# tjuDavidWang/MARL-UAVs-Targets-Tracking

Hardware: NVIDIA B200
Metric: agent-steps/s (higher is better)
Workload: dtype f64

## Files before the change

### marl_uavs_targets_tracking_b200/csrc/common.cuh

```cuda
#pragma once
#include <cuda_runtime.h>
#include <math.h>
#include <stdint.h>
#include <stdio.h>
#include <stdlib.h>
#include <string.h>

#include "../../include/uavsim.h"
#include "philox.cuh"

#define PMI_NT 256

enum { ST_REW, ST_TT, ST_BP, ST_DUP, ST_COV, ST_CMAX, ST_ENVS, ST_PMI_OOR, STAT_W };

static thread_local char g_err[512] = "";
#define SET_ERR(...) snprintf(g_err, sizeof(g_err), __VA_ARGS__)
#define CUDA_TRY(expr)                                                                     \
  do {                                                                                     \
    cudaError_t _e = (expr);                                                               \
    if (_e != cudaSuccess) {                                                               \
      SET_ERR("%s failed: %s (%s:%d)", #expr, cudaGetErrorString(_e), __FILE__, __LINE__); \
      return (int)_e;                                                                      \
    }                                                                                      \
  } while (0)

struct GuardK {
  float t2_up, t2_dn, c1, c0;
};

struct TileBand {
  float r, Cp, Hp, Cd, Hd, Cc, Hc, pad;
};

struct KParams {
  int n, m, na, num_steps;
  int64_t E;
  int64_t env_id_offset;
  double x_max, y_max;
  double dtv_u, dtv_t;
  double dt, uav_h_max;
  double dc, dp, two_dp;
  double tv, uv;
  double tv_over_uv;
  double s_dp_le, s_dp_lt, s_dc_le, s_2dp_le;
  double alpha, beta, gamma;
  double tt_hi;
  double dup_lo;
  double inv_dp, inv_dc, inv_na, inv_tt_hi, inv_dup_span;
  double cx, cy, rmax;
  float f_dp, f_dcmv;
  GuardK g_dp, g_2dp, g_dc, g_pf;
  float r_fast;
  float r_tile;
  TileBand tb[2];
  float dp_f, inv_dp_f, inv_dc_f, inv_na_f, tt_hi_f, inv_tt_hi_f, dup_lo_f, inv_dup_span_f, alpha_f, beta_f, gamma_f;
  float k_ex1_f, tv_over_uv_f, cx_f, cy_f;
  float dtv_u_f;
  const double *sincos_tab;
  int *fast_ctr;
};

struct PmiDev {
  int H;
  const float *w0, *b0, *w1t, *b1, *w2;
  float b2;
};

typedef void (*StepKernelFn)(const KParams, const UavSimBuffers, const double *, int64_t, int64_t, int, int, double,
                             int, long long *);
struct ActEntry;
typedef void (*FastKernelFn)(const KParams, const UavSimBuffers, const ActEntry *, int64_t, int64_t, int, double, int,
                             long long *);

typedef void (*SmallKernelFn)(const KParams, const UavSimBuffers, const ActEntry *, int64_t, int64_t, int, double, int,
                              long long *, int, uint64_t, uint32_t);

struct PmiTcDev;

struct uavsim {
  UavSimParams hp;
  KParams kp;
  UavSimBuffers buf;
  bool bound;
  int device, sm_count;
  int64_t E;
  double *d_dth;
  long long *d_stats;
  double *d_stats8;
  double *h_stats8;
  int stat_slots;
// ... 80 lines not shown
```

### marl_uavs_targets_tracking_b200/csrc/step_fast_kernel.cuh

```cuda
#pragma once
#include "common.cuh"
#include "fast_math.cuh"
#include <stddef.h>
#include "step_kernel.cuh"

#define FAST_NT 64

struct ActEntry {
  double dth;
  float cd, sd;
};

struct __align__(16) SlotRec {
  float4 pos;
  float4 hd;
  float2 a;
  float2 pad;
};
struct __align__(16) TSlot {
  float4 pos;
  float4 vel;
};

template <int N, int M, bool AUX>
struct __align__(128) FastSmem {
  double ux[N], uy[N], uh[N];
  double tx[M], ty[M], th[M];
  int32_t ua[N], act[N];
  double oux[N], ouy[N], ouh[N];
  double otx[M], oty[M], oth[M];
  int32_t oua[N];
  SlotRec slotn[N / 2];
  SlotRec sloto[N / 2];
  TSlot tslot[M / 2];
  double xo[N], yo[N];
  float raw[N];
  int32_t tcnt[AUX ? M : 1];
  uint32_t cover[2][2];
  uint32_t rmax[2];
  unsigned long long mbar;
  long long next_k;
};
static_assert(sizeof(SlotRec) == 48 && sizeof(TSlot) == 32, "slot layout");

__device__ __forceinline__ void sf_expect_tx(uint32_t bar, uint32_t bytes) {
  asm volatile("mbarrier.arrive.expect_tx.shared::cta.b64 _, [%0], %1;" ::"r"(bar), "r"(bytes) : "memory");
}
__device__ __forceinline__ void sf_bulk_g2s(uint32_t dst, const void *src, uint32_t bytes, uint32_t bar) {
  asm volatile("cp.async.bulk.shared::cluster.global.mbarrier::complete_tx::bytes [%0], [%1], %2, [%3];"
               ::"r"(dst), "l"(src), "r"(bytes), "r"(bar) : "memory");
}
__device__ __forceinline__ void sf_bulk_s2g(void *dst, uint32_t src, uint32_t bytes) {
  asm volatile("cp.async.bulk.global.shared::cta.bulk_group [%0], [%1], %2;" ::"l"(dst), "r"(src), "r"(bytes) : "memory");
}
__device__ __forceinline__ uint32_t sf_smem(const void *p) { return (uint32_t)__cvta_generic_to_shared(p); }
__device__ __forceinline__ void sf_mbar_wait(uint32_t bar, uint32_t parity) {
  uint32_t done = 0;
  for (uint32_t spin = 0; !done; spin++) {
    asm volatile(
        "{\n\t.reg .pred P1;\n\t"
        "mbarrier.try_wait.parity.shared::cta.b64 P1, [%1], %2, %3;\n\t"
        "selp.b32 %0, 1, 0, P1;\n\t}"
        : "=r"(done)
        : "r"(bar), "r"(parity), "r"(20000u)
        : "memory");
    if (spin > (1u << 22)) __trap();
  }
}

__device__ __forceinline__ uint64_t f2_sub(uint64_t a, uint64_t b) {
  uint64_t d;
  asm("sub.f32x2 %0, %1, %2;" : "=l"(d) : "l"(a), "l"(b));
  return d;
}
__device__ __forceinline__ uint64_t f2_fma(uint64_t a, uint64_t b, uint64_t c) {
  uint64_t d;
  asm("fma.rn.f32x2 %0, %1, %2, %3;" : "=l"(d) : "l"(a), "l"(b), "l"(c));
  return d;
}
__device__ __forceinline__ uint64_t f2_add(uint64_t a, uint64_t b) {
  uint64_t d;
  asm("add.f32x2 %0, %1, %2;" : "=l"(d) : "l"(a), "l"(b));
  return d;
}
__device__ __forceinline__ uint64_t f2_mul(uint64_t a, uint64_t b) {
  uint64_t d;
  asm("mul.f32x2 %0, %1, %2;" : "=l"(d) : "l"(a), "l"(b));
  return d;
}
__device__ __forceinline__ float f2_lo(uint64_t v) { return __uint_as_float((uint32_t)v); }
__device__ __forceinline__ float f2_hi(uint64_t v) { return __uint_as_float((uint32_t)(v >> 32)); }
__device__ __forceinline__ uint64_t sf_le2(float a0, float a1, float b) {
  uint32_t lo, hi;
  asm("{\n\t.reg .pred p, q;\n\t"
      "setp.le.f32 p, %2, %4;\n\t"
      "setp.le.f32 q, %3, %4;\n\t"
      "selp.b32 %0, 0x3f800000, 0, p;\n\t"
      "selp.b32 %1, 0x3f800000, 0, q;\n\t}"
      : "=r"(lo), "=r"(hi) : "f"(a0), "f"(a1), "f"(b));
  return (uint64_t)lo | ((uint64_t)hi << 32);
}
__device__ __forceinline__ float sf_le(float a, float b) { return (a <= b) ? 1.0f : 0.0f; }
__device__ __forceinline__ int sf_msb(uint32_t w) {
  int r;
  asm("bfind.u32 %0, %1;" : "=r"(r) : "r"(w));
  return r;
}
__device__ __forceinline__ float sf_rcp(float x) {
  float r;
  asm("rcp.approx.ftz.f32 %0, %1;" : "=f"(r) : "f"(x));
  return r;
}

template <bool TWO, int STRIDE>
__device__ __forceinline__ void prefilter64(const void *__restrict__ pf, float xf, float yf, float thrA, float thrB,
                                            uint32_t &aE, uint32_t &aO, uint32_t &bE, uint32_t &bO) {
  const uint64_t xf2 = pack2(xf, xf), yf2 = pack2(yf, yf), nA = pack2(-thrA, -thrA), nB = pack2(-thrB, -thrB);
  const unsigned char *base = reinterpret_cast<const unsigned char *>(pf);
  uint32_t ae = 0, ao = 0, be = 0, bo = 0;
#ifndef FAST_PF_UNROLL
#define FAST_PF_UNROLL 8
#endif
#pragma unroll 1
  for (int k = 0; k < 32; k += FAST_PF_UNROLL) {
#pragma unroll
    for (int u = 0; u < FAST_PF_UNROLL; u++) {
      const ulonglong2 p = *reinterpret_cast<const ulonglong2 *>(base + (k + u) * STRIDE);
      const uint64_t dx = f2_sub(p.x, xf2), dy = f2_sub(p.y, yf2);
      const uint64_t tA = f2_fma(dx, dx, f2_fma(dy, dy, nA));
      ae = __funnelshift_l((uint32_t)tA, ae, 1);
      ao = __funnelshift_l((uint32_t)(tA >> 32), ao, 1);
      if (TWO) {
        const uint64_t tB = f2_fma(dx, dx, f2_fma(dy, dy, nB));
        be = __funnelshift_l((uint32_t)tB, be, 1);
        bo = __funnelshift_l((uint32_t)(tB >> 32), bo, 1);
      }
    }
  }
  aE = __brev(ae); aO = __brev(ao);
// ... 187 lines not shown
      const float dx = r[0] - W.xf, dy = r[2] - W.yf;
      const float s = fmaf(dx, dx, dy * dy);
      if (s > T2_hi) continue;
      if (s > T2_lo && !(sf_exact_pair(S.oux[2 * b + par], S.ouy[2 * b + par], W.xi, W.yi, s_2dp_le, s_2dp_le) & 1)) continue;
      dp[par] |= bit;
      dup += fast_ex2f(fmaf(fast_sqrtf(s), k_ex1, k_ex0));
      if (s <= Tp_hi) {
        bool in = true;
        if (s > Tp_lo) in = sf_exact_pair(S.oux[2 * b + par], S.ouy[2 * b + par], W.xi, W.yi, s_dp_le, s_dp_le) & 1;
        if (in) nb[par] |= bit;
      }
    }
  }
  O->dup = dup; O->nbE = nb[0]; O->nbO = nb[1]; O->dpE = dp[0]; O->dpO = dp[1];
}


#ifndef FAST_LOAD_WARP
#define FAST_LOAD_WARP 1
#endif
#ifndef FAST_COV_THREAD
#define FAST_COV_THREAD 32
#endif
#ifndef FAST_CTAS_PER_SM
#define FAST_CTAS_PER_SM 14
#endif
template <int N, int M, bool AUX>
__global__ void __launch_bounds__(FAST_NT, FAST_CTAS_PER_SM)
uavsim_step_fast_kernel(const KParams P, const UavSimBuffers B, const ActEntry *__restrict__ act_tab, int64_t env_begin,
                        int64_t env_count, int mode, double coop, int done_flag, long long *__restrict__ stats) {
  static_assert(N == 64 && M == 64 && FAST_NT == 64, "one thread per UAV and per target");
  typedef FastSmem<N, M, AUX> SmemT;
  static_assert(offsetof(SmemT, sloto) - offsetof(SmemT, slotn) == sizeof(SlotRec) * (N / 2), "record offset");
  static_assert(sizeof(SlotRec) * N >= sizeof(float) * 12 * N && sizeof(TSlot) * (M / 2) >= sizeof(float) * 4 * N, "output staging");
  extern __shared__ __align__(128) unsigned char fast_smem_raw[];
  SmemT &S = *reinterpret_cast<SmemT *>(fast_smem_raw);
  float *const s_obs = reinterpret_cast<float *>(S.slotn);
  float *const s_rew = reinterpret_cast<float *>(S.tslot);
  const int t = threadIdx.x, lane = t & 31, warp = t >> 5;
  const uint32_t bar = sf_smem(&S.mbar);
  constexpr uint32_t IN_BYTES = 3 * N * 8 + 3 * M * 8 + 2 * N * 4;
  constexpr uint32_t OLD_OFF = (uint32_t)(sizeof(SlotRec) * (N / 2));
  const bool pmi_pending = (mode == UAVSIM_MODE_PMI) && (coop != 0.0);

  auto issue_loads = [&](int64_t e) {
    sf_expect_tx(bar, IN_BYTES);
    sf_bulk_g2s(sf_smem(S.ux), B.ux + e * N, N * 8, bar);
    sf_bulk_g2s(sf_smem(S.uy), B.uy + e * N, N * 8, bar);
    sf_bulk_g2s(sf_smem(S.uh), B.uh + e * N, N * 8, bar);
    sf_bulk_g2s(sf_smem(S.tx), B.tx + e * M, M * 8, bar);
    sf_bulk_g2s(sf_smem(S.ty), B.ty + e * M, M * 8, bar);
    sf_bulk_g2s(sf_smem(S.th), B.th + e * M, M * 8, bar);
    sf_bulk_g2s(sf_smem(S.ua), B.ua + e * N, N * 4, bar);
    sf_bulk_g2s(sf_smem(S.act), B.actions + e * N, N * 4, bar);
  };

  if (t == 0) {
    mbar_init(bar, 1);
    asm volatile("fence.mbarrier_init.release.cluster;" ::: "memory");
  }
  __syncthreads();
  if (warp == 0 && (int64_t)blockIdx.x < env_count) {
    if (elect_one()) issue_loads(env_begin + blockIdx.x);
  }

  const int64_t plane = P.E * N;
  const float inv_dp_f = P.inv_dp_f, inv_dc_f = P.inv_dc_f, inv_na_f = P.inv_na_f;
  const float k_ex0 = 1.4426950408889634f, k_ex1 = P.k_ex1_f;
  int fx_r = 0, fx_tt = 0, fx_bp = 0, fx_dup = 0;
  long long fxs_r = 0, fxs_tt = 0, fxs_bp = 0, fxs_dup = 0;
  long long st_cov = 0, st_envs = 0;
  int st_cmax = 0;
  uint32_t trips = 0;
  uint32_t parity = 0;
  const int ih = t >> 1, ic = t & 1;
  const int ihx = ih + ic;

  for (int64_t k = blockIdx.x, k_next = 0; k < env_count; k = k_next) {
    const int64_t e = env_begin + k;
    sf_mbar_wait(bar, parity);
    parity ^= 1;

    double t_x = S.tx[t], t_y = S.ty[t], t_h = S.th[t];
    float t_vx, t_vy;
    {
      double sh, ch;
      heading_sincos(t_h, P.sincos_tab, sh, ch);
      t_x += P.dtv_t * ch;
      t_y += P.dtv_t * sh;
      if (0 > t_y || t_y > P.y_max) { t_h = -t_h; sh = -sh; }
      else if (t_x < 0 || t_x > P.x_max) { t_h = (t_h > 0) ? (PI_D - t_h) : (-PI_D - t_h); ch = -ch; }
      t_vx = (float)ch * P.tv_over_uv_f; t_vy = (float)sh * P.tv_over_uv_f;
    }
    const float txf = (float)(t_x - P.cx), tyf = (float)(t_y - P.cy);
    float rabs = fmaxf(fabsf(txf), fabsf(tyf));
    double xi, yi, hi;
    float xf, yf, chf, shf, xl, yl;
    const double xo_d = S.ux[t], yo_d = S.uy[t];
    const int a_old = S.ua[t], ai = S.act[t];
    float xof, yof, cof, sof;
    {
      double h = S.uh[t];
      double sh, ch;
      heading_sincos(h, P.sincos_tab, sh, ch);
      cof = (float)ch; sof = (float)sh;
      xof = (float)(xo_d - P.cx); yof = (float)(yo_d - P.cy);
      xi = xo_d + P.dtv_u * ch;
      yi = yo_d + P.dtv_u * sh;
      double dh;
      float cd, sd;
      if ((unsigned)ai < (unsigned)P.na) {
        const ActEntry en = act_tab[ai];
        dh = en.dth; cd = en.cd; sd = en.sd;
      } else {
        dh = P.dt * ((double)(2 * (ai + 1) - P.na - 1) * P.uav_h_max / (double)(P.na - 1));
        double sd_, cd_;
        sincos_shared(dh, &sd_, &cd_);
        cd = (float)cd_; sd = (float)sd_;
      }
      hi = wrap_heading(h + dh);
      chf = fmaf(cof, cd, -(sof * sd));
      shf = fmaf(sof, cd, cof * sd);
      xf = (float)(xi - P.cx); yf = (float)(yi - P.cy);
      xl = (float)((xi - P.cx) - (double)xf); yl = (float)((yi - P.cy) - (double)yf);
      rabs = fmaxf(fmaxf(rabs, fmaxf(fabsf(xf), fabsf(yf))), fmaxf(fabsf(xof), fabsf(yof)));
      if ((unsigned)ai >= 4096u || (unsigned)a_old >= 4096u) rabs = __int_as_float(0x7f800000);
      if (!(rabs == rabs)) rabs = __int_as_float(0x7f800000);
    }
    if (warp == 0) {
      if (elect_one()) asm volatile("cp.async.bulk.wait_group.read 0;" ::: "memory");
    }
    __syncthreads();
    {
      S.otx[t] = t_x; S.oty[t] = t_y; S.oth[t] = t_h;
      float *ts = reinterpret_cast<float *>(&S.tslot[ih]) + ic;
      ts[0] = txf; ts[2] = tyf; ts[4] = t_vx; ts[6] = t_vy;
      if (AUX) S.tcnt[t] = 0;
      S.xo[t] = xo_d; S.yo[t] = yo_d;
      float *so = reinterpret_cast<float *>(&S.sloto[ih]) + ic;
      so[0] = xof; so[2] = yof; so[4] = cof; so[6] = sof; so[8] = (float)a_old;
      S.oux[t] = xi; S.ouy[t] = yi; S.ouh[t] = hi; S.oua[t] = ai;
      float *sn = reinterpret_cast<float *>(&S.slotn[ih]) + ic;
      sn[0] = xf; sn[2] = yf; sn[4] = chf; sn[6] = shf; sn[8] = (float)ai;
    }
    {
      const uint32_t rm = __reduce_max_sync(0xffffffffu, __float_as_uint(rabs));
      if (lane == 0) S.rmax[warp] = rm;
    }
    __syncthreads();
    if (warp == FAST_LOAD_WARP) {
      if (elect_one()) {
        const int64_t kn = (int64_t)gridDim.x + (int64_t)atomicAdd(P.fast_ctr, 1);
        S.next_k = kn;
        if (kn < env_count) issue_loads(env_begin + kn);
      }
    }

    const float R = __uint_as_float(max(S.rmax[0], S.rmax[1]));
    const bool far_env = !(R <= P.r_fast);
    const bool near_origin = fabs(xi) < 2.0 && fabs(yi) < 2.0;
    const int64_t mrow_t = (e * N + t) * M, mrow_u = (e * N + t) * N;
    float o0, o1, o2, o3, o4, o5, o6, o7, o8, tt_f, dup_f;
    uint32_t nbE = 0, nbO = 0, cvE = 0, cvO = 0;
    uint32_t ncE = 0, ncO = 0;
    uint32_t cmE = 0, cmO = 0, dpE = 0, dpO = 0;
#ifdef FAST_ABL_NOPAIRS
    const bool exact = false;
    o0 = o1 = o2 = o3 = o4 = o5 = o6 = o7 = o8 = -1.f; tt_f = 0.f; dup_f = 0.f;
    if (far_env && near_origin) {
#else
    const bool exact = far_env || near_origin;
    if (!exact) {
#endif
      const float g_dp = fmaf(R, P.g_dp.c1, P.g_dp.c0), g_2dp = fmaf(R, P.g_2dp.c1, P.g_2dp.c0);
      const float ndtv_f = -P.dtv_u_f;
      const float g_dc = 2.0f * fmaf(R, P.g_dc.c1, P.g_dc.c0) + P.g_dc.c1 * fabsf(P.dtv_u_f);
      const float g_pf = fmaf(R, P.g_pf.c1, P.g_pf.c0);
      const float Tp_hi = __fadd_ru(P.g_dp.t2_up, g_dp), Tp_lo = __fadd_rd(P.g_dp.t2_dn, -g_dp);
      const float T2_hi = __fadd_ru(P.g_2dp.t2_up, g_2dp), T2_lo = __fadd_rd(P.g_2dp.t2_dn, -g_2dp);
      const float Tc_hi = __fadd_ru(P.g_dc.t2_up, g_dc), Tc_lo = __fadd_rd(P.g_dc.t2_dn, -g_dc);
      const float Tf_hi = __fadd_ru(P.g_pf.t2_up, g_pf);
      const uint64_t xf2 = pack2(xf, xf), yf2 = pack2(yf, yf);
      const WalkOwn WO = {xi, yi, xf, yf, t};

      uint32_t ccE, ccO;
      {
        uint32_t d0, d1;
        prefilter64<false, (int)sizeof(TSlot)>(S.tslot, xf, yf, Tp_hi, 0.f, cvE, cvO, d0, d1);
        float ox = 0, oy = 0, ovx = 0, ovy = 0, ttacc = 0, smax_t = 0;
#pragma unroll
        for (int par = 0; par < 2; par++) {
          uint32_t w = par ? cvO : cvE;
          const float *rec = reinterpret_cast<const float *>(S.tslot) + par;
#pragma unroll 1
          while (w) {
            const int b = sf_msb(w);
            w ^= 1u << b;
            const float *r = rec + 8 * b;
            const float dx = r[0] - xf, dy = r[2] - yf;
            const float s = fmaf(dx, dx, dy * dy);
            smax_t = fmaxf(smax_t, s);
            ox += dx; oy += dy; ovx += r[4]; ovy += r[6];
            ttacc = fmaf(fast_sqrtf(s), -inv_dp_f, ttacc);
          }
        }
        if (smax_t > Tp_lo) {
          TgtOut X;
          sf_targets_checked<N, M, AUX>(&S, WO, Tp_lo, P.s_dp_le, P.s_dp_lt, inv_dp_f, cvE, cvO, &X);
          ox = X.ox; oy = X.oy; ovx = X.ovx; ovy = X.ovy; ttacc = X.ttacc;
          cvE = X.cvE; cvO = X.cvO; ncE = X.ncE; ncO = X.ncO;
        }
        const int nobs = __popc(cvE) + __popc(cvO);
        if (nobs) {
          const float kf = (float)nobs, rk = sf_rcp(kf);
          o5 = fmaf(ox, rk, -xl) * inv_dp_f;
          o6 = fmaf(oy, rk, -yl) * inv_dp_f;
          o7 = fmaf(ovx, rk, -chf);
          o8 = fmaf(ovy, rk, -shf);
          tt_f = fmaf(2.0f, kf, ttacc);
        } else {
          o5 = o6 = o7 = o8 = -1.f;
          tt_f = 0.f;
        }
      }

      uint32_t d0_, d1_;
      prefilter64<false, (int)sizeof(SlotRec)>(S.slotn, xf, yf, Tf_hi, 0.f, ccE, ccO, d0_, d1_);
      const unsigned char *slot_new = reinterpret_cast<const unsigned char *>(S.slotn);
      const unsigned char *slot_old = reinterpret_cast<const unsigned char *>(S.sloto);
      {
        uint64_t sx = 0, sy = 0, sc = 0, ss = 0, sa = 0, cn = 0, dp2 = 0;
        float smax_c = 0.f, smax_d = 0.f, dmin_n = 3.0e38f;
        const float Tp_nx = __uint_as_float(__float_as_uint(Tp_hi) + 1u);
        const uint64_t tpn2 = pack2(Tp_nx, Tp_nx);
        const float nb_band = fmaxf(__fadd_ru(Tp_nx, -Tp_lo), 4.0f * (Tp_nx - Tp_hi));
        const uint64_t kx1 = pack2(k_ex1, k_ex1), kx0 = pack2(k_ex0, k_ex0);
        uint32_t w = ccE | ccO;
#pragma unroll 1
        while (w) {
          const int b = sf_msb(w);
          const uint32_t bit = 1u << b;
// ... 21 lines not shown
          sa = f2_fma(wh, aa, sa);
          cn = f2_add(cn, wh);
          if (AUX) { if (h0) cmE |= bit; if (h1) cmO |= bit; }
          const uint64_t n2 = f2_fma(ex, ex, f2_mul(ey, ey));
          const float n0 = f2_lo(n2), n1 = f2_hi(n2);
          const bool g0 = n0 <= T2_hi, g1 = n1 <= T2_hi;
          const uint64_t wg = pack2(g0 ? 1.0f : 0.0f, g1 ? 1.0f : 0.0f);
          {
            const uint64_t nw = f2_mul(n2, wg);
            smax_d = fmaxf(fmaxf(smax_d, f2_lo(nw)), f2_hi(nw));
          }
          const uint64_t arg = f2_fma(pack2(fast_sqrtf(n0), fast_sqrtf(n1)), kx1, kx0);
          dp2 = f2_fma(wg, pack2(fast_ex2f(f2_lo(arg)), fast_ex2f(f2_hi(arg))), dp2);
          if (AUX) { if (g0) dpE |= bit; if (g1) dpO |= bit; }
          {
            const uint64_t dn = f2_sub(n2, tpn2);
            const uint32_t m0 = (uint32_t)((int32_t)(uint32_t)dn >> 31), m1 = (uint32_t)((int32_t)(uint32_t)(dn >> 32) >> 31);
            nbE |= m0 & bit; nbO |= m1 & bit;
            dmin_n = fminf(fminf(dmin_n, fabsf(f2_lo(dn))), fabsf(f2_hi(dn)));
          }
        }
        float own_w, own_dx, own_dy, own_c, own_s, own_a;
        {
          const float *r = reinterpret_cast<const float *>(slot_new + (ic ? 0u : OLD_OFF) + 48 * ih) + ic;
          own_c = r[4]; own_s = r[6]; own_a = r[8];
          own_dx = own_c * (ic ? 0.0f : ndtv_f); own_dy = own_s * (ic ? 0.0f : ndtv_f);
          const float s_own = fmaf(own_dx, own_dx, own_dy * own_dy);
          own_w = sf_le(s_own, Tc_hi);
        }
        float tsx = f2_lo(sx) + f2_hi(sx), tsy = f2_lo(sy) + f2_hi(sy), tsc = f2_lo(sc) + f2_hi(sc);
        float tss = f2_lo(ss) + f2_hi(ss), tsa = f2_lo(sa) + f2_hi(sa), tcn = f2_lo(cn) + f2_hi(cn);
        if (smax_c > Tc_lo) {
          CommOut X;
          sf_comm_checked<N, M, AUX>(&S, WO, Tc_lo, Tc_hi, P.s_dc_le, ihx, ccE | ccO, &X);
          tsx = X.sx; tsy = X.sy; tsc = X.sc; tss = X.ss; tsa = X.sa; tcn = X.cn;
          if (AUX) { cmE = X.cmE; cmO = X.cmO; }
        }
        const float cntf = tcn - own_w;
        if (AUX) { if (ic) cmO &= ~(1u << ih); else cmE &= ~(1u << ih); }
        if (cntf > 0.5f) {
          const float rk = sf_rcp(cntf);
          o0 = fmaf(tsx - own_w * own_dx, rk, -xl) * inv_dc_f;
          o1 = fmaf(tsy - own_w * own_dy, rk, -yl) * inv_dc_f;
          o2 = fmaf(tsc - own_w * own_c, rk, -chf);
          o3 = fmaf(tss - own_w * own_s, rk, -shf);
          o4 = ((tsa - own_w * own_a) - cntf * (float)ai) * (rk * inv_na_f);
        } else {
          o0 = o1 = o2 = o3 = o4 = -1.f;
        }
        const uint32_t ownE = ic ? 0u : (1u << ih), ownO = ic ? (1u << ih) : 0u;
        float dup = (f2_lo(dp2) + f2_hi(dp2)) - fast_ex2f(fmaf(fast_sqrtf(0.f), k_ex1, k_ex0));
        nbE &= ~ownE; nbO &= ~ownO;
        if (AUX) { dpE &= ~ownE; dpO &= ~ownO; }
        if ((smax_d > T2_lo) || (dmin_n <= nb_band)) {
          DupOut X;
          sf_dup_checked<N, M, AUX>(&S, WO, T2_lo, T2_hi, Tp_lo, Tp_hi, P.s_2dp_le, P.s_dp_le, k_ex0, k_ex1, (ccE | ccO) & ~ownE,
                                    (ccE | ccO) & ~ownO, &X);
          dup = X.dup; nbE = X.nbE; nbO = X.nbO;
          if (AUX) { dpE = X.dpE; dpO = X.dpO; }
        }
        dup_f = -0.5f * dup;
      }
    }
    if (exact) {
      const ExactK XK = {P.s_dp_le, P.s_dp_lt, P.s_2dp_le, P.s_dc_le, P.dp, P.dc, P.two_dp, P.na};
      const MaskPtrs MP = {B.obs_mask, B.comm_mask, B.nbr_mask, B.dup_mask, B.cover_mask};
      FastAgent X;
      fast_agent_exact<N, M, AUX>(XK, MP, S, t, mrow_t, mrow_u, &X);
      o0 = X.ob[0]; o1 = X.ob[1]; o2 = X.ob[2]; o3 = X.ob[3]; o4 = X.ob[4];
      o5 = X.ob[5]; o6 = X.ob[6]; o7 = X.ob[7]; o8 = X.ob[8];
      tt_f = X.tt; dup_f = X.dup;
      nbE = X.nb[0]; nbO = X.nb[1]; cvE = X.cov[0]; cvO = X.cov[1];
    } else if (AUX && B.obs_mask) {
      for (int j = 0; j < 64; j++) {
        const int b = j >> 1;
        const uint8_t v = (((j & 1) ? cvO : cvE) >> b) & 1u;
        B.obs_mask[mrow_t + j] = v; B.cover_mask[mrow_t + j] = v & ~((((j & 1) ? ncO : ncE) >> b) & 1u);
        B.comm_mask[mrow_u + j] = (((j & 1) ? cmO : cmE) >> b) & 1u;
        B.nbr_mask[mrow_u + j] = (((j & 1) ? nbO : nbE) >> b) & 1u;
        B.dup_mask[mrow_u + j] = (((j & 1) ? dpO : dpE) >> b) & 1u;
      }
    }
    cvE &= ~ncE; cvO &= ~ncO;
    if (AUX && B.tracker_cnt) {
#pragma unroll
      for (int par = 0; par < 2; par++) {
        uint32_t w = par ? cvO : cvE;
        while (w) { const int b = sf_msb(w); w ^= 1u << b; atomicAdd(&S.tcnt[2 * b + par], 1); }
      }
    }
    {
      const uint32_t c0 = __reduce_or_sync(0xffffffffu, cvE), c1 = __reduce_or_sync(0xffffffffu, cvO);
      if (lane == 0) { S.cover[warp][0] = c0; S.cover[warp][1] = c1; }
    }

    float raw, ttn, bpn, dupn;
    {
      const float dbdr = fminf(P.cx_f - fabsf(xf), P.cy_f - fabsf(yf));
      bool inside = dbdr > 0.f;
      if (fabsf(dbdr) < 1e-3f) inside = 0 <= xi && xi <= P.x_max && 0 <= yi && yi <= P.y_max;
      const float bp = inside ? ((dbdr < P.dp_f) ? (-0.5f * (P.dp_f - dbdr) * inv_dp_f) : 0.0f) : -0.5f;
      ttn = fminf(fmaxf(tt_f, 0.0f), P.tt_hi_f) * P.inv_tt_hi_f;
      dupn = (fminf(fmaxf(dup_f, P.dup_lo_f), 0.0f) - P.dup_lo_f) * P.inv_dup_span_f - 1.0f;
      bpn = (fminf(fmaxf(bp, -0.5f), 0.0f) + 0.5f) * 2.0f - 1.0f;
      raw = fmaf(P.alpha_f, ttn, fmaf(P.beta_f, bpn, P.gamma_f * dupn));
      S.raw[t] = raw;
    }
    __syncthreads();
    k_next = S.next_k;

    {
      float *ob = s_obs + t * 12;
      reinterpret_cast<float4 *>(ob)[0] = make_float4(o0, o1, o2, o3);
      reinterpret_cast<float4 *>(ob)[1] = make_float4(o4, o5, o6, o7);
      reinterpret_cast<float4 *>(ob)[2] = make_float4(o8, (float)(xi * P.inv_dc), (float)(yi * P.inv_dc), (float)ai * inv_na_f);
      float r;
      const int64_t gi = e * N + t;
      if (mode == UAVSIM_MODE_SELF || coop == 0.0) {
        r = raw;
      } else if (mode == UAVSIM_MODE_MEAN) {
        float s = 0;
        const int cnt = __popc(nbE) + __popc(nbO);
        {
          uint32_t u = nbE | nbO;
          float s1 = 0;
          while (u) {
            const int b = sf_msb(u);
            const uint32_t bit = 1u << b;
            u ^= bit;
            const float2 rr = *reinterpret_cast<const float2 *>(&S.raw[2 * b]);
            s += (nbE & bit) ? rr.x : 0.0f;
            s1 += (nbO & bit) ? rr.y : 0.0f;
          }
          s += s1;
        }
        const float cf = (float)coop;
        r = cnt ? fmaf(1.0f - cf, raw, cf * s * sf_rcp((float)cnt)) : 0.0f;
      } else {
        r = 0.0f;
        B.raw[gi] = (double)raw;
        B.nbr_bits[gi * 2] = sf_interleave(nbE, nbO);
        B.nbr_bits[gi * 2 + 1] = 0;
      }
      r = fminf(fmaxf(r, -1.0f), 1.0f);
      s_rew[t] = r;
      s_rew[N + t] = ttn;
      s_rew[2 * N + t] = bpn;
      s_rew[3 * N + t] = dupn;
      if (!pmi_pending) fx_r += sf_fx(r);
      fx_tt += sf_fx(ttn); fx_bp += sf_fx(bpn); fx_dup += sf_fx(dupn);
      if ((++trips & 255u) == 0u) {
        fxs_r += fx_r; fxs_tt += fx_tt; fxs_bp += fx_bp; fxs_dup += fx_dup;
        fx_r = fx_tt = fx_bp = fx_dup = 0;
      }
      if (AUX && B.tracker_cnt) B.tracker_cnt[e * M + t] = S.tcnt[t];
    }
    asm volatile("fence.proxy.async.shared::cta;" ::: "memory");
    __syncthreads();
    if (warp == 0) {
      if (elect_one()) {
        sf_bulk_s2g(B.ux + e * N, sf_smem(S.oux), N * 8);
        sf_bulk_s2g(B.uy + e * N, sf_smem(S.ouy), N * 8);
        sf_bulk_s2g(B.uh + e * N, sf_smem(S.ouh), N * 8);
        sf_bulk_s2g(B.ua + e * N, sf_smem(S.oua), N * 4);
        sf_bulk_s2g(B.tx + e * M, sf_smem(S.otx), M * 8);
        sf_bulk_s2g(B.ty + e * M, sf_smem(S.oty), M * 8);
        sf_bulk_s2g(B.th + e * M, sf_smem(S.oth), M * 8);
        sf_bulk_s2g(B.obs + e * N * 12, sf_smem(s_obs), N * 48);
        if (!pmi_pending) sf_bulk_s2g(B.rew4 + e * N, sf_smem(s_rew), N * 4);
        sf_bulk_s2g(B.rew4 + plane + e * N, sf_smem(s_rew + N), N * 4);
        sf_bulk_s2g(B.rew4 + 2 * plane + e * N, sf_smem(s_rew + 2 * N), N * 4);
        sf_bulk_s2g(B.rew4 + 3 * plane + e * N, sf_smem(s_rew + 3 * N), N * 4);
        asm volatile("cp.async.bulk.commit_group;" ::: "memory");
      }
    }
    if (t == FAST_COV_THREAD) {
      const int c = __popc(S.cover[0][0] | S.cover[1][0]) + __popc(S.cover[0][1] | S.cover[1][1]);
      B.covered[e] = c;
      if (B.done) B.done[e] = done_flag;
      st_cov += c;
      st_cmax = max(st_cmax, c);
      st_envs++;
    }
  }
  __syncwarp();
  if (warp == 0) {
    if (elect_one()) asm volatile("cp.async.bulk.wait_group 0;" ::: "memory");
  }
  work_counter_leave(P.fast_ctr);
  stats_commit(stats + (size_t)blockIdx.x * STAT_W, fxs_r + fx_r, fxs_tt + fx_tt, fxs_bp + fx_bp, fxs_dup + fx_dup, st_cov,
               st_cmax, st_envs);
}
```

### marl_uavs_targets_tracking_b200/csrc/uavsim.cu

```cuda
#include <cfloat>
#include <cmath>
#include <mutex>
#include <vector>

#include "common.cuh"
#include "step_kernel.cuh"
#include "pmi_kernel.cuh"
#include "pmi_tc_kernel.cuh"
#include "step_fast_kernel.cuh"
#include "step_tile_kernel.cuh"
#include "step_small_kernel.cuh"
#include "aux_kernels.cuh"
#include "replay.cuh"

static double exact_sq_threshold(double thr, bool strict) {
  double s = thr * thr;
  auto ok = [&](double v) { double r = sqrt(v); return strict ? (r < thr) : (r <= thr); };
  while (!ok(s)) s = nextafter(s, -INFINITY);
  while (ok(nextafter(s, INFINITY))) s = nextafter(s, INFINITY);
  return s;
}

static int raise_dynamic_smem(const void *fn, int device, size_t bytes) {
  static struct { const void *fn; int device; size_t bytes; } seen[256];
// ... 117 lines not shown
  k.g_dc = make_guard(p->dc, k.rmax);
  {
    const double rmin = p->dp < p->dc ? p->dp : p->dc;
    double rf = 2e-6 * 16777216.0 * rmin;
    if (rf > k.rmax) rf = k.rmax;
    k.r_fast = (float)rf;
    k.r_tile = (float)(rf < 4096.0 ? rf : 4096.0);
    const double cmax = k.cx > k.cy ? k.cx : k.cy;
    const double rr[2] = {1.3 * cmax < k.r_tile ? 1.3 * cmax : (double)k.r_tile, (double)k.r_tile};
    for (int lv = 0; lv < 2; lv++) {
      auto band = [&](const GuardK &G, float &C, float &H) {
        const double gd = ((double)G.c1 * rr[lv] + (double)G.c0) * (1.0 + 1e-6);
        const double hi = (double)G.t2_up + gd, lo = (double)G.t2_dn - gd;
        C = (float)(0.5 * (hi + lo));
        const double hw = 0.5 * (hi - lo) + 2.4e-7 * fabs(hi) + fabs((double)C - 0.5 * (hi + lo));
        H = nextafterf((float)hw, INFINITY);
        if ((double)H < hw) H = nextafterf(H, INFINITY);
      };
      k.tb[lv].r = (float)rr[lv];
      if ((double)k.tb[lv].r > rr[lv]) k.tb[lv].r = nextafterf(k.tb[lv].r, 0.f);
      band(k.g_dp, k.tb[lv].Cp, k.tb[lv].Hp);
      band(k.g_2dp, k.tb[lv].Cd, k.tb[lv].Hd);
      band(k.g_dc, k.tb[lv].Cc, k.tb[lv].Hc);
      k.tb[lv].pad = 0.f;
    }
  }
  k.dp_f = (float)p->dp; k.inv_dp_f = (float)k.inv_dp; k.inv_dc_f = (float)k.inv_dc; k.inv_na_f = (float)k.inv_na;
  k.tt_hi_f = (float)k.tt_hi; k.inv_tt_hi_f = (float)k.inv_tt_hi; k.dup_lo_f = (float)k.dup_lo; k.inv_dup_span_f = (float)k.inv_dup_span;
  k.alpha_f = (float)k.alpha; k.beta_f = (float)k.beta; k.gamma_f = (float)k.gamma;
  k.k_ex1_f = (float)(-1.4426950408889634 / k.two_dp); k.tv_over_uv_f = (float)k.tv_over_uv;
  k.cx_f = (float)k.cx; k.cy_f = (float)k.cy;
  k.dtv_u_f = (float)k.dtv_u;
  {
    double tab[FM_TAB_SIZE * 2];
    fm_fill_table(tab);
    CUDA_TRY(cudaMalloc(&h->d_sctab, sizeof(tab)));
    CUDA_TRY(cudaMemcpy(h->d_sctab, tab, sizeof(tab), cudaMemcpyHostToDevice));
    k.sincos_tab = h->d_sctab;
    CUDA_TRY(cudaMalloc(&h->d_fast_ctr, 2 * sizeof(int)));
    CUDA_TRY(cudaMemset(h->d_fast_ctr, 0, 2 * sizeof(int)));
    k.fast_ctr = h->d_fast_ctr;
  }

  std::vector<double> dth_v(3 * (size_t)p->na);
  double *dth = dth_v.data();
  for (int a = 0; a < p->na; a++) {
    const int na1 = a + 1;
    const double rate = (double)(2 * na1 - p->na - 1) * p->uav_h_max / (double)(p->na - 1);
    dth[3 * a] = p->dt * rate;
    dth[3 * a + 1] = cos(dth[3 * a]);
    dth[3 * a + 2] = sin(dth[3 * a]);
  }
  CUDA_TRY(cudaMalloc(&h->d_dth, sizeof(double) * 3 * p->na));
  CUDA_TRY(cudaMemcpy(h->d_dth, dth, sizeof(double) * 3 * p->na, cudaMemcpyHostToDevice));
  {
    std::vector<ActEntry> tab(p->na);
    for (int a = 0; a < p->na; a++) { tab[a].dth = dth[3 * a]; tab[a].cd = (float)dth[3 * a + 1]; tab[a].sd = (float)dth[3 * a + 2]; }
    CUDA_TRY(cudaMalloc(&h->d_act, sizeof(ActEntry) * p->na));
    CUDA_TRY(cudaMemcpy(h->d_act, tab.data(), sizeof(ActEntry) * p->na, cudaMemcpyHostToDevice));
  }

  if (k.n == 64 && k.m == 64) { h->nt = UAVSIM_NT64; h->step_fn[0] = uavsim_step_kernel<64, 64, false, UAVSIM_NT64>; h->step_fn[1] = uavsim_step_kernel<64, 64, true, UAVSIM_NT64>; }
  else if (k.n == 10 && k.m == 10) { h->nt = 128; h->step_fn[0] = uavsim_step_kernel<10, 10, false, 128>; h->step_fn[1] = uavsim_step_kernel<10, 10, true, 128>; }
  else { h->nt = 128; h->step_fn[0] = uavsim_step_kernel<0, 0, false, 128>; h->step_fn[1] = uavsim_step_kernel<0, 0, true, 128>; }
  int epb = h->nt / p->n_uav;
  if (epb < 1) epb = 1;
  const bool fixed_shape = (k.n == 64 && k.m == 64) || (k.n == 10 && k.m == 10);
  if (!fixed_shape) {
    if ((int64_t)epb > n_envs) epb = (int)n_envs;
    while (epb > 1 && step_smem_bytes(k.n, k.m, k.na, epb) > 64 * 1024) epb--;
  }
  h->epb = epb;
  h->smem_step = step_smem_bytes(k.n, k.m, k.na, epb);
  if (h->smem_step > 227 * 1024) {
    SET_ERR("uavsim_create: n_uav=%d m_targets=%d needs %zu B shared memory per CTA", k.n, k.m, h->smem_step);
    return UAVSIM_ERR_UNSUPPORTED;
  }
  for (int v = 0; v < 2; v++) {
    int rc = raise_dynamic_smem((const void *)h->step_fn[v], device, h->smem_step);
    if (rc) return rc;
  }
  int occ = 1;
  CUDA_TRY(cudaOccupancyMaxActiveBlocksPerMultiprocessor(&occ, h->step_fn[0], h->nt, h->smem_step));
  if (occ < 1) occ = 1;
  h->grid_max = h->sm_count * occ;
  h->has_fast = (k.n == 64 && k.m == 64);
  if (h->has_fast) {
    h->fast_fn[0] = uavsim_step_fast_kernel<64, 64, false>;
    h->fast_fn[1] = uavsim_step_fast_kernel<64, 64, true>;
    h->smem_fast[0] = sizeof(FastSmem<64, 64, false>);
    h->smem_fast[1] = sizeof(FastSmem<64, 64, true>);
    for (int v = 0; v < 2; v++) {
      int rc = raise_dynamic_smem((const void *)h->fast_fn[v], device, h->smem_fast[v]);
      if (rc) return rc;
      int o = 1;
      CUDA_TRY(cudaOccupancyMaxActiveBlocksPerMultiprocessor(&o, h->fast_fn[v], FAST_NT, h->smem_fast[v]));
      h->fast_grid_max[v] = h->sm_count * (o < 1 ? 1 : o);
      if (h->fast_grid_max[v] > h->grid_max) h->grid_max = h->fast_grid_max[v];
    }
    h->tile_fn[0] = uavsim_step_tile_kernel<false>;
    h->tile_fn[1] = uavsim_step_tile_kernel<true>;
    h->smem_tile[0] = sizeof(TileSmem<false>);
    h->smem_tile[1] = sizeof(TileSmem<true>);
    for (int v = 0; v < 2; v++) {
      int rc = raise_dynamic_smem((const void *)h->tile_fn[v], device, h->smem_tile[v]);
      if (rc) return rc;
      int o = 1;
      CUDA_TRY(cudaOccupancyMaxActiveBlocksPerMultiprocessor(&o, h->tile_fn[v], TILE_NT, h->smem_tile[v]));
      h->tile_grid_max[v] = h->sm_count * (o < 1 ? 1 : o);
      if (h->tile_grid_max[v] > h->grid_max) h->grid_max = h->tile_grid_max[v];
    }
  }
  h->has_small = (k.n <= SMALL_MAX && k.m <= SMALL_MAX);
  int small_warps = 0;
  if (h->has_small) {
    h->small_fn[0] = uavsim_step_small_kernel<false>;
    h->small_fn[1] = uavsim_step_small_kernel<true>;
    for (int v = 0; v < 2; v++) {
      int o = 1;
      CUDA_TRY(cudaOccupancyMaxActiveBlocksPerMultiprocessor(&o, h->small_fn[v], SMALL_NT, 0));
      h->small_grid_max[v] = h->sm_count * (o < 1 ? 1 : o);
      if (h->small_grid_max[v] > small_warps) small_warps = h->small_grid_max[v];
    }
  }
// ... 634 lines not shown
```

Measured before the change: 10.09 billion.

## Add strip-grid target culling, smem action table, and reduce register pressure in fast kernel

Replaces the full 64-target prefilter scan with a per-env 1D strip grid on x and y. Each target sets bits in overlapping strip windows, and each UAV only tests targets whose bits survive in both its x and y strips. The action table moves into shared memory, per-thread stat accumulators become per-warp shared counters updated by warp reductions, and several live values (env index, own position, lane-local data) are reloaded from shared memory instead of held in registers. The likely aim is to cut per-UAV distance work and register pressure. The cost is shared atomics, extra syncs on strip zeroing, and more dynamic shared memory, which may lower occupancy.

```diff
diff --git a/marl_uavs_targets_tracking_b200/csrc/common.cuh b/marl_uavs_targets_tracking_b200/csrc/common.cuh
--- a/marl_uavs_targets_tracking_b200/csrc/common.cuh
+++ b/marl_uavs_targets_tracking_b200/csrc/common.cuh
@@ -56,6 +56,8 @@
   float dp_f, inv_dp_f, inv_dc_f, inv_na_f, tt_hi_f, inv_tt_hi_f, dup_lo_f, inv_dup_span_f, alpha_f, beta_f, gamma_f;
   float k_ex1_f, tv_over_uv_f, cx_f, cy_f;
   float dtv_u_f;
+  float tg_q, tg_inv_x, tg_off_x, tg_inv_y, tg_off_y;
+  int tg_nx, tg_ny;
   const double *sincos_tab;
   int *fast_ctr;
 };
diff --git a/marl_uavs_targets_tracking_b200/csrc/step_fast_kernel.cuh b/marl_uavs_targets_tracking_b200/csrc/step_fast_kernel.cuh
--- a/marl_uavs_targets_tracking_b200/csrc/step_fast_kernel.cuh
+++ b/marl_uavs_targets_tracking_b200/csrc/step_fast_kernel.cuh
@@ -5,6 +5,7 @@
 #include "step_kernel.cuh"
 
 #define FAST_NT 64
+#define FAST_STRIPS 32
 
 struct ActEntry {
   double dth;
@@ -33,6 +34,7 @@
   SlotRec slotn[N / 2];
   SlotRec sloto[N / 2];
   TSlot tslot[M / 2];
+  uint2 xwin[FAST_STRIPS], ywin[FAST_STRIPS];
   double xo[N], yo[N];
   float raw[N];
   int32_t tcnt[AUX ? M : 1];
@@ -40,6 +42,10 @@
   uint32_t rmax[2];
   unsigned long long mbar;
   long long next_k;
+  long long cur_e;
+  long long fx[2][4];
+  long long cov_sum;
+  int cov_max, n_env;
 };
 static_assert(sizeof(SlotRec) == 48 && sizeof(TSlot) == 32, "slot layout");
 
@@ -105,6 +111,9 @@
   int r;
   asm("bfind.u32 %0, %1;" : "=r"(r) : "r"(w));
   return r;
+}
+__device__ __forceinline__ int sf_strip(float u, float inv, float off, int nc) {
+  return min(max(__float2int_rd(fmaf(u, inv, off)), 0), nc - 1);
 }
 __device__ __forceinline__ float sf_rcp(float x) {
   float r;
@@ -358,6 +367,8 @@
   static_assert(N == 64 && M == 64 && FAST_NT == 64, "one thread per UAV and per target");
   typedef FastSmem<N, M, AUX> SmemT;
   static_assert(offsetof(SmemT, sloto) - offsetof(SmemT, slotn) == sizeof(SlotRec) * (N / 2), "record offset");
+  static_assert(offsetof(SmemT, xwin) % 16 == 0 && offsetof(SmemT, ywin) == offsetof(SmemT, xwin) + 8 * FAST_STRIPS &&
+                2 * FAST_STRIPS * 8 <= 16 * FAST_NT, "strip windows are zeroed with one 16-byte store per thread");
   static_assert(sizeof(SlotRec) * N >= sizeof(float) * 12 * N && sizeof(TSlot) * (M / 2) >= sizeof(float) * 4 * N, "output staging");
   extern __shared__ __align__(128) unsigned char fast_smem_raw[];
   SmemT &S = *reinterpret_cast<SmemT *>(fast_smem_raw);
@@ -381,6 +392,11 @@
     sf_bulk_g2s(sf_smem(S.act), B.actions + e * N, N * 4, bar);
   };
 
+  ActEntry *const s_act = reinterpret_cast<ActEntry *>(fast_smem_raw + sizeof(SmemT));
+  for (int a = t; a < P.na; a += FAST_NT) s_act[a] = act_tab[a];
+  if (t < FAST_STRIPS) reinterpret_cast<uint4 *>(S.xwin)[t] = make_uint4(0, 0, 0, 0);
+  if (lane == 0) for (int k = 0; k < 4; k++) S.fx[warp][k] = 0;
+  if (t == FAST_COV_THREAD) { S.cov_sum = 0; S.cov_max = 0; S.n_env = 0; }
   if (t == 0) {
     mbar_init(bar, 1);
     asm volatile("fence.mbarrier_init.release.cluster;" ::: "memory");
@@ -393,17 +409,11 @@
   const int64_t plane = P.E * N;
   const float inv_dp_f = P.inv_dp_f, inv_dc_f = P.inv_dc_f, inv_na_f = P.inv_na_f;
   const float k_ex0 = 1.4426950408889634f, k_ex1 = P.k_ex1_f;
-  int fx_r = 0, fx_tt = 0, fx_bp = 0, fx_dup = 0;
-  long long fxs_r = 0, fxs_tt = 0, fxs_bp = 0, fxs_dup = 0;
-  long long st_cov = 0, st_envs = 0;
-  int st_cmax = 0;
-  uint32_t trips = 0;
   uint32_t parity = 0;
   const int ih = t >> 1, ic = t & 1;
   const int ihx = ih + ic;
 
   for (int64_t k = blockIdx.x, k_next = 0; k < env_count; k = k_next) {
-    const int64_t e = env_begin + k;
     sf_mbar_wait(bar, parity);
     parity ^= 1;
 
@@ -421,6 +431,7 @@
     const float txf = (float)(t_x - P.cx), tyf = (float)(t_y - P.cy);
     float rabs = fmaxf(fabsf(txf), fabsf(tyf));
     double xi, yi, hi;
+    bool near_origin;
     float xf, yf, chf, shf, xl, yl;
     const double xo_d = S.ux[t], yo_d = S.uy[t];
     const int a_old = S.ua[t], ai = S.act[t];
@@ -436,7 +447,7 @@
       double dh;
       float cd, sd;
       if ((unsigned)ai < (unsigned)P.na) {
-        const ActEntry en = act_tab[ai];
+        const ActEntry en = s_act[ai];
         dh = en.dth; cd = en.cd; sd = en.sd;
       } else {
         dh = P.dt * ((double)(2 * (ai + 1) - P.na - 1) * P.uav_h_max / (double)(P.na - 1));
@@ -449,6 +460,7 @@
       shf = fmaf(sof, cd, cof * sd);
       xf = (float)(xi - P.cx); yf = (float)(yi - P.cy);
       xl = (float)((xi - P.cx) - (double)xf); yl = (float)((yi - P.cy) - (double)yf);
+      near_origin = fabs(xi) < 2.0 && fabs(yi) < 2.0;
       rabs = fmaxf(fmaxf(rabs, fmaxf(fabsf(xf), fabsf(yf))), fmaxf(fabsf(xof), fabsf(yof)));
       if ((unsigned)ai >= 4096u || (unsigned)a_old >= 4096u) rabs = __int_as_float(0x7f800000);
       if (!(rabs == rabs)) rabs = __int_as_float(0x7f800000);
@@ -458,9 +470,22 @@
     }
     __syncthreads();
     {
+      if (t == 0) S.cur_e = env_begin + k;
       S.otx[t] = t_x; S.oty[t] = t_y; S.oth[t] = t_h;
       float *ts = reinterpret_cast<float *>(&S.tslot[ih]) + ic;
       ts[0] = txf; ts[2] = tyf; ts[4] = t_vx; ts[6] = t_vy;
+      {
+        const float q = P.tg_q;
+        const uint32_t bit = 1u << ih;
+        const int gx1 = sf_strip(txf + q, P.tg_inv_x, P.tg_off_x, P.tg_nx);
+#pragma unroll 1
+        for (int g = sf_strip(txf - q, P.tg_inv_x, P.tg_off_x, P.tg_nx); g <= gx1; g++)
+          atomicOr(reinterpret_cast<uint32_t *>(&S.xwin[g]) + ic, bit);
+        const int gy1 = sf_strip(tyf + q, P.tg_inv_y, P.tg_off_y, P.tg_ny);
+#pragma unroll 1
+        for (int g = sf_strip(tyf - q, P.tg_inv_y, P.tg_off_y, P.tg_ny); g <= gy1; g++)
+          atomicOr(reinterpret_cast<uint32_t *>(&S.ywin[g]) + ic, bit);
+      }
       if (AUX) S.tcnt[t] = 0;
       S.xo[t] = xo_d; S.yo[t] = yo_d;
       float *so = reinterpret_cast<float *>(&S.sloto[ih]) + ic;
@@ -484,8 +509,7 @@
 
     const float R = __uint_as_float(max(S.rmax[0], S.rmax[1]));
     const bool far_env = !(R <= P.r_fast);
-    const bool near_origin = fabs(xi) < 2.0 && fabs(yi) < 2.0;
-    const int64_t mrow_t = (e * N + t) * M, mrow_u = (e * N + t) * N;
+    const float *const own_new = reinterpret_cast<const float *>(&S.slotn[ih]) + ic;
     float o0, o1, o2, o3, o4, o5, o6, o7, o8, tt_f, dup_f;
     uint32_t nbE = 0, nbO = 0, cvE = 0, cvO = 0;
     uint32_t ncE = 0, ncO = 0;
@@ -507,12 +531,27 @@
       const float Tc_hi = __fadd_ru(P.g_dc.t2_up, g_dc), Tc_lo = __fadd_rd(P.g_dc.t2_dn, -g_dc);
       const float Tf_hi = __fadd_ru(P.g_pf.t2_up, g_pf);
       const uint64_t xf2 = pack2(xf, xf), yf2 = pack2(yf, yf);
-      const WalkOwn WO = {xi, yi, xf, yf, t};
+      auto own_walk = [&]() { return WalkOwn{S.oux[t], S.ouy[t], xf, yf, t}; };
 
       uint32_t ccE, ccO;
       {
-        uint32_t d0, d1;
-        prefilter64<false, (int)sizeof(TSlot)>(S.tslot, xf, yf, Tp_hi, 0.f, cvE, cvO, d0, d1);
+        {
+          const uint2 wx = S.xwin[sf_strip(xf, P.tg_inv_x, P.tg_off_x, P.tg_nx)];
+          const uint2 wy = S.ywin[sf_strip(yf, P.tg_inv_y, P.tg_off_y, P.tg_ny)];
+          const uint64_t nT = pack2(-Tp_hi, -Tp_hi);
+          uint32_t w = (wx.x & wy.x) | (wx.y & wy.y);
+#pragma unroll 1
+          while (w) {
+            const int b = sf_msb(w);
+            const uint32_t bit = 1u << b;
+            w ^= bit;
+            const ulonglong2 p = *reinterpret_cast<const ulonglong2 *>(&S.tslot[b].pos);
+            const uint64_t dx = f2_sub(p.x, xf2), dy = f2_sub(p.y, yf2);
+            const uint64_t tA = f2_fma(dx, dx, f2_fma(dy, dy, nT));
+            cvE |= (uint32_t)((int32_t)(uint32_t)tA >> 31) & bit;
+            cvO |= (uint32_t)((int32_t)(uint32_t)(tA >> 32) >> 31) & bit;
+          }
+        }
         float ox = 0, oy = 0, ovx = 0, ovy = 0, ttacc = 0, smax_t = 0;
 #pragma unroll
         for (int par = 0; par < 2; par++) {
@@ -532,7 +571,7 @@
         }
         if (smax_t > Tp_lo) {
           TgtOut X;
-          sf_targets_checked<N, M, AUX>(&S, WO, Tp_lo, P.s_dp_le, P.s_dp_lt, inv_dp_f, cvE, cvO, &X);
+          sf_targets_checked<N, M, AUX>(&S, own_walk(), Tp_lo, P.s_dp_le, P.s_dp_lt, inv_dp_f, cvE, cvO, &X);
           ox = X.ox; oy = X.oy; ovx = X.ovx; ovy = X.ovy; ttacc = X.ttacc;
           cvE = X.cvE; cvO = X.cvO; ncE = X.ncE; ncO = X.ncO;
         }
@@ -620,7 +659,7 @@
         float tss = f2_lo(ss) + f2_hi(ss), tsa = f2_lo(sa) + f2_hi(sa), tcn = f2_lo(cn) + f2_hi(cn);
         if (smax_c > Tc_lo) {
           CommOut X;
-          sf_comm_checked<N, M, AUX>(&S, WO, Tc_lo, Tc_hi, P.s_dc_le, ihx, ccE | ccO, &X);
+          sf_comm_checked<N, M, AUX>(&S, own_walk(), Tc_lo, Tc_hi, P.s_dc_le, ihx, ccE | ccO, &X);
           tsx = X.sx; tsy = X.sy; tsc = X.sc; tss = X.ss; tsa = X.sa; tcn = X.cn;
           if (AUX) { cmE = X.cmE; cmO = X.cmO; }
         }
@@ -628,11 +667,12 @@
         if (AUX) { if (ic) cmO &= ~(1u << ih); else cmE &= ~(1u << ih); }
         if (cntf > 0.5f) {
           const float rk = sf_rcp(cntf);
-          o0 = fmaf(tsx - own_w * own_dx, rk, -xl) * inv_dc_f;
-          o1 = fmaf(tsy - own_w * own_dy, rk, -yl) * inv_dc_f;
-          o2 = fmaf(tsc - own_w * own_c, rk, -chf);
-          o3 = fmaf(tss - own_w * own_s, rk, -shf);
-          o4 = ((tsa - own_w * own_a) - cntf * (float)ai) * (rk * inv_na_f);
+          const float xl2 = (float)((S.oux[t] - P.cx) - (double)xf), yl2 = (float)((S.ouy[t] - P.cy) - (double)yf);
+          o0 = fmaf(tsx - own_w * own_dx, rk, -xl2) * inv_dc_f;
+          o1 = fmaf(tsy - own_w * own_dy, rk, -yl2) * inv_dc_f;
+          o2 = fmaf(tsc - own_w * own_c, rk, -own_new[4]);
+          o3 = fmaf(tss - own_w * own_s, rk, -own_new[6]);
+          o4 = ((tsa - own_w * own_a) - cntf * own_new[8]) * (rk * inv_na_f);
         } else {
           o0 = o1 = o2 = o3 = o4 = -1.f;
         }
@@ -642,7 +682,7 @@
         if (AUX) { dpE &= ~ownE; dpO &= ~ownO; }
         if ((smax_d > T2_lo) || (dmin_n <= nb_band)) {
           DupOut X;
-          sf_dup_checked<N, M, AUX>(&S, WO, T2_lo, T2_hi, Tp_lo, Tp_hi, P.s_2dp_le, P.s_dp_le, k_ex0, k_ex1, (ccE | ccO) & ~ownE,
+          sf_dup_checked<N, M, AUX>(&S, own_walk(), T2_lo, T2_hi, Tp_lo, Tp_hi, P.s_2dp_le, P.s_dp_le, k_ex0, k_ex1, (ccE | ccO) & ~ownE,
                                     (ccE | ccO) & ~ownO, &X);
           dup = X.dup; nbE = X.nbE; nbO = X.nbO;
           if (AUX) { dpE = X.dpE; dpO = X.dpO; }
@@ -650,6 +690,8 @@
         dup_f = -0.5f * dup;
       }
     }
+    const int64_t e = S.cur_e;
+    const int64_t mrow_t = (e * N + t) * M, mrow_u = (e * N + t) * N;
     if (exact) {
       const ExactK XK = {P.s_dp_le, P.s_dp_lt, P.s_2dp_le, P.s_dc_le, P.dp, P.dc, P.two_dp, P.na};
       const MaskPtrs MP = {B.obs_mask, B.comm_mask, B.nbr_mask, B.dup_mask, B.cover_mask};
@@ -683,6 +725,7 @@
     }
 
     float raw, ttn, bpn, dupn;
+    xi = S.oux[t]; yi = S.ouy[t];
     {
       const float dbdr = fminf(P.cx_f - fabsf(xf), P.cy_f - fabsf(yf));
       bool inside = dbdr > 0.f;
@@ -696,12 +739,13 @@
     }
     __syncthreads();
     k_next = S.next_k;
+    if (t < FAST_STRIPS) reinterpret_cast<uint4 *>(S.xwin)[t] = make_uint4(0, 0, 0, 0);
 
     {
       float *ob = s_obs + t * 12;
       reinterpret_cast<float4 *>(ob)[0] = make_float4(o0, o1, o2, o3);
       reinterpret_cast<float4 *>(ob)[1] = make_float4(o4, o5, o6, o7);
-      reinterpret_cast<float4 *>(ob)[2] = make_float4(o8, (float)(xi * P.inv_dc), (float)(yi * P.inv_dc), (float)ai * inv_na_f);
+      reinterpret_cast<float4 *>(ob)[2] = make_float4(o8, (float)(xi * P.inv_dc), (float)(yi * P.inv_dc), (float)S.oua[t] * inv_na_f);
       float r;
       const int64_t gi = e * N + t;
       if (mode == UAVSIM_MODE_SELF || coop == 0.0) {
@@ -735,11 +779,11 @@
       s_rew[N + t] = ttn;
       s_rew[2 * N + t] = bpn;
       s_rew[3 * N + t] = dupn;
-      if (!pmi_pending) fx_r += sf_fx(r);
-      fx_tt += sf_fx(ttn); fx_bp += sf_fx(bpn); fx_dup += sf_fx(dupn);
-      if ((++trips & 255u) == 0u) {
-        fxs_r += fx_r; fxs_tt += fx_tt; fxs_bp += fx_bp; fxs_dup += fx_dup;
-        fx_r = fx_tt = fx_bp = fx_dup = 0;
+      {
+        const int w_r = __reduce_add_sync(0xffffffffu, pmi_pending ? 0 : sf_fx(r));
+        const int w_tt = __reduce_add_sync(0xffffffffu, sf_fx(ttn)), w_bp = __reduce_add_sync(0xffffffffu, sf_fx(bpn));
+        const int w_dup = __reduce_add_sync(0xffffffffu, sf_fx(dupn));
+        if (lane == 0) { S.fx[warp][0] += w_r; S.fx[warp][1] += w_tt; S.fx[warp][2] += w_bp; S.fx[warp][3] += w_dup; }
       }
       if (AUX && B.tracker_cnt) B.tracker_cnt[e * M + t] = S.tcnt[t];
     }
@@ -747,28 +791,31 @@
     __syncthreads();
     if (warp == 0) {
       if (elect_one()) {
-        sf_bulk_s2g(B.ux + e * N, sf_smem(S.oux), N * 8);
-        sf_bulk_s2g(B.uy + e * N, sf_smem(S.ouy), N * 8);
-        sf_bulk_s2g(B.uh + e * N, sf_smem(S.ouh), N * 8);
-        sf_bulk_s2g(B.ua + e * N, sf_smem(S.oua), N * 4);
-        sf_bulk_s2g(B.tx + e * M, sf_smem(S.otx), M * 8);
-        sf_bulk_s2g(B.ty + e * M, sf_smem(S.oty), M * 8);
-        sf_bulk_s2g(B.th + e * M, sf_smem(S.oth), M * 8);
-        sf_bulk_s2g(B.obs + e * N * 12, sf_smem(s_obs), N * 48);
-        if (!pmi_pending) sf_bulk_s2g(B.rew4 + e * N, sf_smem(s_rew), N * 4);
-        sf_bulk_s2g(B.rew4 + plane + e * N, sf_smem(s_rew + N), N * 4);
-        sf_bulk_s2g(B.rew4 + 2 * plane + e * N, sf_smem(s_rew + 2 * N), N * 4);
-        sf_bulk_s2g(B.rew4 + 3 * plane + e * N, sf_smem(s_rew + 3 * N), N * 4);
+        const int64_t o = S.cur_e * N;
+        sf_bulk_s2g(B.ux + o, sf_smem(S.oux), N * 8);
+        sf_bulk_s2g(B.uy + o, sf_smem(S.ouy), N * 8);
+        sf_bulk_s2g(B.uh + o, sf_smem(S.ouh), N * 8);
+        sf_bulk_s2g(B.ua + o, sf_smem(S.oua), N * 4);
+        sf_bulk_s2g(B.tx + o, sf_smem(S.otx), M * 8);
+        sf_bulk_s2g(B.ty + o, sf_smem(S.oty), M * 8);
+        sf_bulk_s2g(B.th + o, sf_smem(S.oth), M * 8);
+        sf_bulk_s2g(B.obs + o * 12, sf_smem(s_obs), N * 48);
+        float *const rw = B.rew4 + o;
+        if (!pmi_pending) sf_bulk_s2g(rw, sf_smem(s_rew), N * 4);
+        sf_bulk_s2g(rw + plane, sf_smem(s_rew + N), N * 4);
+        sf_bulk_s2g(rw + 2 * plane, sf_smem(s_rew + 2 * N), N * 4);
+        sf_bulk_s2g(rw + 3 * plane, sf_smem(s_rew + 3 * N), N * 4);
         asm volatile("cp.async.bulk.commit_group;" ::: "memory");
       }
     }
     if (t == FAST_COV_THREAD) {
       const int c = __popc(S.cover[0][0] | S.cover[1][0]) + __popc(S.cover[0][1] | S.cover[1][1]);
-      B.covered[e] = c;
-      if (B.done) B.done[e] = done_flag;
-      st_cov += c;
-      st_cmax = max(st_cmax, c);
-      st_envs++;
+      const int64_t ec = S.cur_e;
+      B.covered[ec] = c;
+      if (B.done) B.done[ec] = done_flag;
+      S.cov_sum += c;
+      S.cov_max = max(S.cov_max, c);
+      S.n_env++;
     }
   }
   __syncwarp();
@@ -776,6 +823,7 @@
     if (elect_one()) asm volatile("cp.async.bulk.wait_group 0;" ::: "memory");
   }
   work_counter_leave(P.fast_ctr);
-  stats_commit(stats + (size_t)blockIdx.x * STAT_W, fxs_r + fx_r, fxs_tt + fx_tt, fxs_bp + fx_bp, fxs_dup + fx_dup, st_cov,
-               st_cmax, st_envs);
-}
+  const bool ct = t == FAST_COV_THREAD, l0 = lane == 0;
+  stats_commit(stats + (size_t)blockIdx.x * STAT_W, l0 ? S.fx[warp][0] : 0, l0 ? S.fx[warp][1] : 0, l0 ? S.fx[warp][2] : 0,
+               l0 ? S.fx[warp][3] : 0, ct ? S.cov_sum : 0, ct ? S.cov_max : 0, ct ? S.n_env : 0);
+}
diff --git a/marl_uavs_targets_tracking_b200/csrc/uavsim.cu b/marl_uavs_targets_tracking_b200/csrc/uavsim.cu
--- a/marl_uavs_targets_tracking_b200/csrc/uavsim.cu
+++ b/marl_uavs_targets_tracking_b200/csrc/uavsim.cu
@@ -173,6 +173,24 @@
   k.cx_f = (float)k.cx; k.cy_f = (float)k.cy;
   k.dtv_u_f = (float)k.dtv_u;
   {
+    const double tmax = ((double)k.g_dp.t2_up + (double)k.g_dp.c1 * (double)k.r_fast + (double)k.g_dp.c0) * (1.0 + 0x1p-20);
+    float c = (float)(sqrt(tmax) * (1.0 + 0x1p-20));
+    while ((double)c * (double)c < tmax) c = nextafterf(c, INFINITY);
+    const double q = (double)c + ((double)k.r_fast + (double)c) * 0x1p-22;
+    k.tg_q = (float)q;
+    if ((double)k.tg_q < q) k.tg_q = nextafterf(k.tg_q, INFINITY);
+    auto axis = [&](double ext, double centre, int &nc, float &inv, float &off) {
+      double w = 0.5 * (double)k.tg_q;
+      if (w < ext / FAST_STRIPS) w = ext / FAST_STRIPS;
+      const double cnt = ceil(ext / w);
+      nc = cnt < 1 ? 1 : (cnt > FAST_STRIPS ? FAST_STRIPS : (int)cnt);
+      inv = (float)(1.0 / w);
+      off = (float)(centre / w);
+    };
+    axis(p->x_max, k.cx, k.tg_nx, k.tg_inv_x, k.tg_off_x);
+    axis(p->y_max, k.cy, k.tg_ny, k.tg_inv_y, k.tg_off_y);
+  }
+  {
     double tab[FM_TAB_SIZE * 2];
     fm_fill_table(tab);
     CUDA_TRY(cudaMalloc(&h->d_sctab, sizeof(tab)));
@@ -225,12 +243,13 @@
   CUDA_TRY(cudaOccupancyMaxActiveBlocksPerMultiprocessor(&occ, h->step_fn[0], h->nt, h->smem_step));
   if (occ < 1) occ = 1;
   h->grid_max = h->sm_count * occ;
-  h->has_fast = (k.n == 64 && k.m == 64);
+  const size_t act_bytes = sizeof(ActEntry) * (size_t)p->na;
+  h->has_fast = (k.n == 64 && k.m == 64) && sizeof(FastSmem<64, 64, true>) + act_bytes <= 227 * 1024;
   if (h->has_fast) {
     h->fast_fn[0] = uavsim_step_fast_kernel<64, 64, false>;
     h->fast_fn[1] = uavsim_step_fast_kernel<64, 64, true>;
-    h->smem_fast[0] = sizeof(FastSmem<64, 64, false>);
-    h->smem_fast[1] = sizeof(FastSmem<64, 64, true>);
+    h->smem_fast[0] = sizeof(FastSmem<64, 64, false>) + act_bytes;
+    h->smem_fast[1] = sizeof(FastSmem<64, 64, true>) + act_bytes;
     for (int v = 0; v < 2; v++) {
       int rc = raise_dynamic_smem((const void *)h->fast_fn[v], device, h->smem_fast[v]);
       if (rc) return rc;
```

Result: faster. 10.63 billion, median of 6 (+5.3%).
